# cropinghigh/sdrpp-dvbs-demodulator

Hardware: NVIDIA B200
Metric: decoded_info_gbit_s (higher is better)
Workload: dtype int8

## Files before the change

sdrpp-dvbs-demodulator_b200/csrc/api.cu:

```cuda
#include "../../include/dvbs2fec.h"

#include <algorithm>
#include <atomic>
#include <chrono>
#include <climits>
#include <condition_variable>
#include <cstdarg>
#include <cstdio>
#include <cstring>
#include <deque>
#include <map>
#include <memory>
#include <mutex>
#include <string>
#include <thread>
#include <vector>

#include <cuda_runtime.h>
#include <emmintrin.h>

#include "bch_decoder.cuh"
#include "demapper.cuh"
#include "host_tables.h"
#include "ldpc_decoder.cuh"
// ... 10 lines not shown
    va_start(ap, fmt);
    vsnprintf(g_err, sizeof(g_err), fmt, ap);
    va_end(ap);
    return code;
}
}
namespace s2 {
int api_fail(int code, const char* msg) {
    snprintf(g_err, sizeof(g_err), "%s", msg);
    return code;
}
}
namespace {
#define CU(call)                                                                              \
    do {                                                                                      \
        cudaError_t e_ = (call);                                                              \
        if (e_ != cudaSuccess)                                                                \
            return fail(DVBS2FEC_ECUDA, "%s: %s (%s:%d)", #call, cudaGetErrorString(e_), __FILE__, __LINE__); \
    } while (0)

constexpr int kStages = 4;
constexpr int kPiece = 256;
constexpr int kSlots = 2;

template <typename T>
struct DevBuf {
    T* p = nullptr;
    size_t cap = 0;
    cudaError_t reserve(size_t n) {
        if (n <= cap) return cudaSuccess;
        if (p) cudaFree(p);
        p = nullptr;
        cap = 0;
        cudaError_t e = cudaMalloc(&p, n * sizeof(T));
        if (e == cudaSuccess) cap = n;
        return e;
    }
    void release() {
        if (p) cudaFree(p);
        p = nullptr;
        cap = 0;
    }
};
template <typename T>
struct PinBuf {
    T* p = nullptr;
// ... 12 lines not shown
        p = nullptr;
        cap = 0;
    }
};

struct Slot {
    cudaStream_t stream = nullptr;
    cudaEvent_t done = nullptr;
    cudaStream_t copy = nullptr;
    cudaEvent_t armed = nullptr;
    DevBuf<unsigned int> arrived;
    DevBuf<uint8_t> ts;
    DevBuf<int> ts_len;
    PinBuf<unsigned int> arrived_vals;
    DevBuf<int8_t> llr;
    DevBuf<float> sym;
    DevBuf<uint8_t> idx;
    DevBuf<uint8_t> hard;
    DevBuf<int16_t> iters;
    DevBuf<int16_t> corr;
    DevBuf<uint8_t> bb;
    DevBuf<dvbs2fec_result> res;
    DevBuf<uint8_t> workspace;
    DevBuf<unsigned int> counter;
    PinBuf<uint8_t> h_in;
    PinBuf<uint8_t> h_bb;
    PinBuf<dvbs2fec_result> h_res;
    uint8_t* user_bb = nullptr;
    dvbs2fec_result* user_res = nullptr;
    int pending = 0;
    bool staged_out = true;
    uint64_t tag_base = 0;
};

struct CodeDev {
    DevBuf<uint8_t> row_level;
};
struct BchTabDev {
    DevBuf<uint16_t> crc, basis;
};

struct DevCtx {
    int device = 0;
    int sms = 0;
    Slot slot[2 * kSlots + 1];
    std::mutex dev_mu;
    bool dev_used = false;
    std::map<int, CodeDev> codes;
    std::map<int, BchTabDev> bch;
    DevBuf<uint16_t> gf_log[2], gf_exp[2];
    DevBuf<uint8_t> prbs;
    DevBuf<uint8_t> pl_rn;
    std::map<int, DevBuf<uint32_t>> luts;
    LdpcDev ldpc{};
    BchDev bchd{};
    DemapDev demap{};
    int grid = 0;
    ~DevCtx() { ldpc_release(ldpc); }
};

}

struct dvbs2fec_ts_parser {
    int device = 0;
    int kb = 0, max_dfl = 0;
    cudaStream_t stream = nullptr;
    DevBuf<TsState> state;
    DevBuf<TsPlan> plan;
    DevBuf<uint32_t> meta;
    DevBuf<uint8_t> bb, out;
    PinBuf<int> h_produced;
    int gse_pool = 0;
    DevBuf<GseState> gstate;
    DevBuf<uint8_t> gbuf, g_sync;
    DevBuf<int> g_doff, g_before, g_nxt, g_aux, g_aux2;
// ... 130 lines not shown
    D.lut = nullptr;
    D.rn = h->pl_codenum >= 0 ? d.pl_rn.p : nullptr;
    if (mc.constellation != APSK32) {
        int key = (mc.constellation == APSK16) ? mc.modcod : (int)mc.constellation;
        DevBuf<uint32_t>& lut = d.luts[key];
        if (!lut.p) {
            std::vector<uint32_t> tab = demap_lut(ch);
            CU(lut.reserve(tab.size()));
            CU(cudaMemcpy(lut.p, tab.data(), tab.size() * 4, cudaMemcpyHostToDevice));
            CU(cudaStreamSynchronize(nullptr));
        }
        D.lut = lut.p;
    }
    return 0;
}

size_t input_frame_bytes(const dvbs2fec_handle* h, int kind) {
    return kind == 1 ? (size_t)h->plsyms * 8 : kind == 2 ? (size_t)(h->code->N / h->mc.bits) * 2 : (size_t)h->code->N;
}

int reserve_slot(dvbs2fec_handle* h, DevCtx& d, Slot& s, int nframes, int kind, bool host_staging) {
    const LdpcCode& c = *h->code;
    CU(cudaSetDevice(d.device));
    CU(s.llr.reserve((size_t)nframes * c.N));
    if (kind == 1) CU(s.sym.reserve((size_t)nframes * h->plsyms * 2));
    if (kind == 2) CU(s.idx.reserve((size_t)nframes * input_frame_bytes(h, 2)));
    CU(s.hard.reserve((size_t)nframes * h->hard_stride));
    CU(s.iters.reserve(nframes));
    CU(s.corr.reserve(nframes));
    CU(s.bb.reserve((size_t)nframes * (c.kbch / 8)));
    CU(s.res.reserve(nframes));
    CU(s.workspace.reserve((size_t)d.grid * ldpc_workspace_bytes(d.ldpc)));
    CU(s.counter.reserve(1));
    if (host_staging) {
        size_t in_bytes = (size_t)nframes * input_frame_bytes(h, kind);
        CU(s.h_in.reserve(in_bytes));
        CU(s.h_bb.reserve((size_t)nframes * (c.kbch / 8)));
        CU(s.h_res.reserve(nframes));
    }
    return 0;
}

int enqueue_chain(dvbs2fec_handle* h, DevCtx& d, Slot& s, const float* d_sym, const int8_t* d_llr, int n,
                  uint8_t* d_bb, dvbs2fec_result* d_res, cudaStream_t st, int* launches, uint64_t tag_base = 0,
                  const unsigned int* arrived = nullptr, const uint8_t* d_idx = nullptr) {
    const int8_t* llr = d_llr;
    dvbs2fec_handle::Span cur{0, nullptr, nullptr};
    auto mark = [&](int kind, bool begin) {
        if (!h->profiling) return;
        if (begin) {
            cur = dvbs2fec_handle::Span{kind, nullptr, nullptr};
            cudaEventCreate(&cur.a);
            cudaEventCreate(&cur.b);
            cudaEventRecord(cur.a, st);
        } else {
            cudaEventRecord(cur.b, st);
            std::lock_guard<std::mutex> lk(h->span_mu);
            h->spans.push_back(cur);
        }
    };
    if (d_sym || d_idx) {
        mark(0, true);
        int e = d_sym ? demap_launch(d.demap, d_sym, n, s.llr.p, st) : demap_idx_launch(d.demap, d_idx, n, s.llr.p, st);
        mark(0, false);
        if (e) return fail(DVBS2FEC_ECUDA, "demap launch: %s", cudaGetErrorString((cudaError_t)e));
        llr = s.llr.p;
        ++*launches;
    }
    CU(cudaMemsetAsync(s.counter.p, 0, sizeof(unsigned int), st));
    LdpcArgs la{};
    la.code = d.ldpc;
    la.llr_in = llr;
    la.nframes = n;
    la.max_trials = h->max_trials;
    la.hard_out = s.hard.p;
    la.hard_stride = h->hard_stride;
    la.iters_out = s.iters.p;
    la.llr_out = nullptr;
    la.workspace = s.workspace.p;
    la.work_counter = s.counter.p;
    la.arrived = arrived;
    int grid = std::min(d.grid, (n + 1) / 2);
    mark(1, true);
    int e = ldpc_launch(la, grid, st);
    mark(1, false);
    if (e) return fail(DVBS2FEC_ECUDA, "ldpc launch: %s", cudaGetErrorString((cudaError_t)e));
    ++*launches;
    BchArgs ba{};
    ba.code = d.bchd;
    ba.hard = s.hard.p;
    ba.hard_stride = h->hard_stride;
    ba.nframes = n;
    ba.ldpc_iters = s.iters.p;
    ba.tags = nullptr;
    ba.tag_base = tag_base;
    ba.bb_out = d_bb;
    ba.results = d_res;
    ba.corr_out = nullptr;
    ba.descramble = 1;
    mark(2, true);
    e = bch_launch(ba, st);
    mark(2, false);
    if (e) return fail(DVBS2FEC_ECUDA, "bch launch: %s", cudaGetErrorString((cudaError_t)e));
    ++*launches;
    return 0;
}

int arm_streamed_input(Slot& s, int nframes) {
    CU(s.arrived.reserve(1));
    CU(s.arrived_vals.reserve((size_t)(nframes + kPiece - 1) / kPiece + 1));
    CU(cudaMemsetAsync(s.arrived.p, 0, sizeof(unsigned int), s.copy));
    CU(cudaEventRecord(s.armed, s.copy));
    CU(cudaStreamWaitEvent(s.stream, s.armed, 0));
    return 0;
}
int feed_streamed_input(Slot& s, const uint8_t* src, int nframes, size_t frame_bytes, bool src_pinned) {
    for (int f0 = 0, k = 0; f0 < nframes; f0 += kPiece, ++k) {
        const int n = std::min(kPiece, nframes - f0);
        const uint8_t* from = src + (size_t)f0 * frame_bytes;
        if (!src_pinned) {
            memcpy(s.h_in.p + (size_t)f0 * frame_bytes, from, (size_t)n * frame_bytes);
            from = s.h_in.p + (size_t)f0 * frame_bytes;
        }
        CU(cudaMemcpyAsync(s.llr.p + (size_t)f0 * frame_bytes, from, (size_t)n * frame_bytes, cudaMemcpyHostToDevice, s.copy));
        s.arrived_vals.p[k] = (unsigned int)(f0 + n);
// ... 317 lines not shown
    if (h->worker.joinable()) h->worker.join();
    for (auto& dp : h->devs) {
        DevCtx& d = *dp;
        cudaSetDevice(d.device);
        cudaDeviceSynchronize();
        for (int k = 0; k < 2 * kSlots + 1; ++k) {
            Slot& s = d.slot[k];
            s.llr.release(); s.sym.release(); s.idx.release(); s.hard.release(); s.iters.release(); s.corr.release();
            s.bb.release(); s.res.release(); s.workspace.release(); s.counter.release();
            s.h_in.release(); s.h_bb.release(); s.h_res.release();
            s.arrived.release(); s.arrived_vals.release();
            s.ts.release(); s.ts_len.release();
            if (s.done) cudaEventDestroy(s.done);
            if (s.armed) cudaEventDestroy(s.armed);
            if (s.copy && !(k >= 1 && k < kSlots)) cudaStreamDestroy(s.copy);
            if (s.stream) cudaStreamDestroy(s.stream);
        }
        for (auto& kv : d.codes) kv.second.row_level.release();
        for (auto& kv : d.bch) { kv.second.crc.release(); kv.second.basis.release(); }
        for (auto& kv : d.luts) kv.second.release();
        for (int i = 0; i < 2; ++i) { d.gf_log[i].release(); d.gf_exp[i].release(); }
        d.prbs.release();
        d.pl_rn.release();
    }
    if (h->ts) dvbs2fec_ts_destroy(h->ts);
    if (h->ts_done) cudaEventDestroy(h->ts_done);
    for (auto& sp : h->spans) {
        cudaEventDestroy(sp.a);
        cudaEventDestroy(sp.b);
    }
    for (auto& S : h->stages) {
        S.in.release();
        S.bb.release();
        S.res.release();
        S.ts.release();
        S.ts_len.release();
    }
    delete h;
}

int dvbs2fec_set_modcod(dvbs2fec_handle* h, int modcod, int shortframes, int pilots, int max_trials) {
    if (!h) return fail(DVBS2FEC_EINVAL, "handle is NULL");
    ModcodCfg mc;
    if (!modcod_config(modcod, shortframes != 0, pilots != 0, &mc))
        return fail(DVBS2FEC_EINVAL, "MODCOD %d is outside 1..28", modcod);
    if (mc.code < 0)
// ... 25 lines not shown
    if (codenum > 262141) return fail(DVBS2FEC_EINVAL, "Gold code number %d outside 0..262141", codenum);
    drain_queue(h);
    h->pl_codenum = codenum < 0 ? -1 : codenum;
    for (auto& dp : h->devs) {
        DevCtx& d = *dp;
        CU(cudaSetDevice(d.device));
        if (codenum >= 0) {
            std::vector<uint8_t> rn = pl_scrambling_rn(codenum, 32400 + 36 * 22 + 8);
            CU(d.pl_rn.reserve(rn.size()));
            CU(cudaMemcpy(d.pl_rn.p, rn.data(), rn.size(), cudaMemcpyHostToDevice));
            CU(cudaStreamSynchronize(nullptr));
        }
        d.demap.rn = codenum >= 0 ? d.pl_rn.p : nullptr;
    }
    return 0;
}

int dvbs2fec_kbch(const dvbs2fec_handle* h) { return (h && h->configured) ? h->code->kbch : DVBS2FEC_EINVAL; }
int dvbs2fec_kldpc(const dvbs2fec_handle* h) { return (h && h->configured) ? h->code->K : DVBS2FEC_EINVAL; }
int dvbs2fec_nldpc(const dvbs2fec_handle* h) { return (h && h->configured) ? h->code->N : DVBS2FEC_EINVAL; }
int dvbs2fec_plframe_symbols(const dvbs2fec_handle* h) { return (h && h->configured) ? h->plsyms : DVBS2FEC_EINVAL; }
int dvbs2fec_last_launch_count(const dvbs2fec_handle* h) { return h ? h->last_launches : 0; }

int dvbs2fec_set_profiling(dvbs2fec_handle* h, int on) {
    if (!h) return fail(DVBS2FEC_EINVAL, "handle is NULL");
    h->profiling = on != 0;
    return 0;
}
int dvbs2fec_kernel_times(dvbs2fec_handle* h, float* demap_ms, float* ldpc_ms, float* bch_ms, int* launches) {
    if (!h) return fail(DVBS2FEC_EINVAL, "handle is NULL");
    float acc[3] = {0, 0, 0};
    int n = 0;
    std::vector<dvbs2fec_handle::Span> spans;
    {
        std::lock_guard<std::mutex> lk(h->span_mu);
        spans.swap(h->spans);
    }
    for (auto& sp : spans) {
        float ms = 0;
        CU(cudaEventSynchronize(sp.b));
        CU(cudaEventElapsedTime(&ms, sp.a, sp.b));
        acc[sp.kind] += ms;
        cudaEventDestroy(sp.a);
        cudaEventDestroy(sp.b);
        ++n;
    }
    if (demap_ms) *demap_ms = acc[0];
    if (ldpc_ms) *ldpc_ms = acc[1];
    if (bch_ms) *bch_ms = acc[2];
    if (launches) *launches = n;
    return 0;
}

int dvbs2fec_bb_to_soft(dvbs2fec_handle* h, const float* plframes, int n, int8_t* llr_out) {
    if (!h || !h->configured || !plframes || !llr_out || n < 0) return fail(DVBS2FEC_EINVAL, "bad arguments");
    if (n == 0) return 0;
    DevCtx& d = *h->devs[0];
    Slot& s = d.slot[0];
    int rc = reserve_slot(h, d, s, n, 1, false);
    if (rc) return rc;
    CU(cudaMemcpyAsync(s.sym.p, plframes, (size_t)n * h->plsyms * 8, cudaMemcpyHostToDevice, s.stream));
    int e = demap_launch(d.demap, s.sym.p, n, s.llr.p, s.stream);
    if (e) return fail(DVBS2FEC_ECUDA, "demap launch: %s", cudaGetErrorString((cudaError_t)e));
    CU(cudaMemcpyAsync(llr_out, s.llr.p, (size_t)n * h->code->N, cudaMemcpyDeviceToHost, s.stream));
    CU(cudaStreamSynchronize(s.stream));
    return 0;
}

int dvbs2fec_ldpc_decode(dvbs2fec_handle* h, int8_t* frames, int n, int max_trials, int16_t* iters) {
    if (!h || !h->configured || !frames || n < 0) return fail(DVBS2FEC_EINVAL, "bad arguments");
    if (n == 0) return 0;
    DevCtx& d = *h->devs[0];
    Slot& s = d.slot[0];
    int rc = reserve_slot(h, d, s, n, 0, false);
    if (rc) return rc;
    const size_t bytes = (size_t)n * h->code->N;
    CU(cudaMemcpyAsync(s.llr.p, frames, bytes, cudaMemcpyHostToDevice, s.stream));
    CU(cudaMemsetAsync(s.counter.p, 0, sizeof(unsigned int), s.stream));
    LdpcArgs la{};
    la.code = d.ldpc;
    la.llr_in = s.llr.p;
    la.nframes = n;
    la.max_trials = max_trials > 0 ? max_trials : h->max_trials;
    la.hard_out = s.hard.p;
    la.hard_stride = h->hard_stride;
    la.iters_out = s.iters.p;
    la.llr_out = s.llr.p;
    la.workspace = s.workspace.p;
    la.work_counter = s.counter.p;
    la.arrived = nullptr;
    int e = ldpc_launch(la, std::min(d.grid, (n + 1) / 2), s.stream);
    if (e) return fail(DVBS2FEC_ECUDA, "ldpc launch: %s", cudaGetErrorString((cudaError_t)e));
    CU(cudaMemcpyAsync(frames, s.llr.p, bytes, cudaMemcpyDeviceToHost, s.stream));
    if (iters) CU(cudaMemcpyAsync(iters, s.iters.p, (size_t)n * 2, cudaMemcpyDeviceToHost, s.stream));
    CU(cudaStreamSynchronize(s.stream));
    return 0;
}

int dvbs2fec_bch_decode(dvbs2fec_handle* h, uint8_t* frames, int n, int16_t* corrections) {
    if (!h || !h->configured || !frames || n < 0) return fail(DVBS2FEC_EINVAL, "bad arguments");
    if (n == 0) return 0;
    DevCtx& d = *h->devs[0];
    Slot& s = d.slot[0];
    int rc = reserve_slot(h, d, s, n, 0, false);
    if (rc) return rc;
    const size_t nb = h->code->K / 8;
    CU(cudaMemsetAsync(s.hard.p, 0, (size_t)n * h->hard_stride, s.stream));
    CU(cudaMemcpy2DAsync(s.hard.p, h->hard_stride, frames, nb, nb, n, cudaMemcpyHostToDevice, s.stream));
    BchArgs ba{};
    ba.code = d.bchd;
    ba.hard = s.hard.p;
    ba.hard_stride = h->hard_stride;
    ba.nframes = n;
    ba.corr_out = s.corr.p;
    int e = bch_launch(ba, s.stream);
// ... 616 lines not shown
```

sdrpp-dvbs-demodulator_b200/csrc/bch_decoder.cu:

```cuda
#include "bch_decoder.cuh"

namespace s2 {
namespace {

constexpr int kWarps = 4;
constexpr int kMaxT = 12;

struct ResultRec {
    unsigned long long tag;
    short ldpc_iters;
    short bch_corr;
    unsigned int flags;
};

__device__ __forceinline__ uint32_t gf_mul(const GfDev& f, uint32_t a, uint32_t b) {
    if (!a || !b) return 0;
    int s = (int)f.log[a] + (int)f.log[b];
    if (s >= f.N) s -= f.N;
    return f.exp[s];
}
__device__ __forceinline__ uint32_t gf_div(const GfDev& f, uint32_t a, uint32_t b) {
    if (!a) return 0;
    int s = (int)f.log[a] - (int)f.log[b];
    if (s < 0) s += f.N;
    return f.exp[s];
}
__device__ __forceinline__ uint32_t gf_mul_exp(const GfDev& f, uint32_t a, int e) {
    if (!a) return 0;
    int s = (int)f.log[a] + e;
    if (s >= f.N) s -= f.N;
    return f.exp[s];
}

__device__ __forceinline__ uint32_t warp_xor(uint32_t v) {
#pragma unroll
    for (int o = 16; o; o >>= 1) v ^= __shfl_xor_sync(0xFFFFFFFFu, v, o);
    return v;
}

__global__ void __launch_bounds__(kWarps * 32) bch_kernel(const __grid_constant__ BchArgs a) {
    extern __shared__ __align__(16) uint8_t smem[];
    const BchDev& c = a.code;
    const GfDev& f = c.gf;
    const int t = c.t, NR = 2 * c.t, m = f.m;
    uint16_t* s_crc = reinterpret_cast<uint16_t*>(smem);
    uint16_t* s_basis = s_crc + kMaxT * 256;
    uint8_t* s_frames = reinterpret_cast<uint8_t*>(s_basis + kMaxT * 16);
    const int wid = threadIdx.x >> 5, lane = threadIdx.x & 31;
    uint8_t* fr = s_frames + (size_t)wid * a.hard_stride;
    __shared__ uint16_t s_synd[kWarps][24];
    __shared__ uint16_t s_lambda[kWarps][26];
    __shared__ uint16_t s_ev[kWarps][26];
    __shared__ int s_loc[kWarps][26];
    __shared__ int s_nloc[kWarps];

    for (int x = threadIdx.x; x < t * 256; x += blockDim.x) s_crc[x] = c.crc[x];
    for (int x = threadIdx.x; x < t * 16; x += blockDim.x) s_basis[x] = c.basis[x];
    __syncthreads();

    const int nbytes = c.nbch >> 3, kbytes = c.kbch >> 3;
    for (int frame = blockIdx.x * kWarps + wid; frame < a.nframes; frame += gridDim.x * kWarps) {
        uint8_t* gfr = a.hard + (size_t)frame * a.hard_stride;
        for (int x = lane; x < a.hard_stride / 16; x += 32)
            reinterpret_cast<uint4*>(fr)[x] = reinterpret_cast<const uint4*>(gfr)[x];
        __syncwarp();

        const int chunk = (nbytes + 31) >> 5;
        const int beg = min(lane * chunk, nbytes), end = min(beg + chunk, nbytes);
        uint32_t r[kMaxT];
#pragma unroll
        for (int k = 0; k < kMaxT; ++k) r[k] = 0;
        const uint32_t rmask = (1u << m) - 1u;
        for (int x = beg; x < end; ++x) {
            uint32_t byte = fr[x];
#pragma unroll
            for (int k = 0; k < kMaxT; ++k)
                if (k < t) {
                    uint32_t idx = r[k] >> (m - 8);
// ... 172 lines not shown
            int it = a.ldpc_iters ? a.ldpc_iters[frame] : 0;
            if (a.corr_out) a.corr_out[frame] = (int16_t)corr;
            if (a.results) {
                ResultRec rr;
                rr.tag = a.tags ? a.tags[frame] : a.tag_base + (unsigned long long)frame;
                rr.ldpc_iters = (short)it;
                rr.bch_corr = (short)corr;
                rr.flags = (it < 0 ? 1u : 0u) | (corr < 0 ? 2u : 0u);
                if (a.descramble) {
                    uint32_t crc = 0;
                    for (int n = 0; n < 80; ++n) {
                        uint32_t byte = fr[n >> 3] ^ c.prbs[n >> 3];
                        uint32_t b = ((byte >> (7 - (n & 7))) & 1u) ^ (crc & 1u);
                        crc >>= 1;
                        if (b) crc ^= 0xABu;
                    }
                    if (crc) rr.flags |= 4u;
                }
                reinterpret_cast<ResultRec*>(a.results)[frame] = rr;
            }
        }
        __syncwarp();
    }
}

__global__ void descramble_kernel(uint8_t* frames, int stride, int nframes, int kbytes, const uint8_t* prbs) {
    int x = blockIdx.x * blockDim.x + threadIdx.x;
    int f = blockIdx.y;
    if (x < kbytes && f < nframes) frames[(size_t)f * stride + x] ^= prbs[x];
}

}

int bch_launch(const BchArgs& a, cudaStream_t stream) {
    if (a.nframes <= 0) return 0;
    if (a.code.t > kMaxT || (a.hard_stride & 15)) return (int)cudaErrorInvalidValue;
    size_t smem = (size_t)kMaxT * 256 * 2 + kMaxT * 16 * 2 + (size_t)kWarps * a.hard_stride;
    int grid = (a.nframes + kWarps - 1) / kWarps;
    if (grid > 148 * 16) grid = 148 * 16;
    bch_kernel<<<grid, kWarps * 32, smem, stream>>>(a);
    return (int)cudaGetLastError();
}

int descramble_launch(uint8_t* frames, int stride, int nframes, int kbch, const uint8_t* prbs, cudaStream_t stream) {
    if (nframes <= 0) return 0;
    int kbytes = kbch / 8;
    dim3 grid((kbytes + 255) / 256, nframes);
    descramble_kernel<<<grid, 256, 0, stream>>>(frames, stride, nframes, kbytes, prbs);
    return (int)cudaGetLastError();
}

}
```

sdrpp-dvbs-demodulator_b200/csrc/bch_decoder.cuh:

```cuda
#pragma once
#include <cstdint>
#include <cuda_runtime.h>

namespace s2 {

struct GfDev {
    int m, N;
    const uint16_t* log;
    const uint16_t* exp;
};

struct BchDev {
    GfDev gf;
    int t;
    int nbch, kbch;
    int prefix;
    const uint16_t* crc;
    const uint16_t* basis;
    const uint8_t* prbs;
};

struct BchArgs {
    BchDev code;
    uint8_t* hard;
    int hard_stride;
    int nframes;
    const int16_t* ldpc_iters;
    const uint64_t* tags;
    unsigned long long tag_base;
    uint8_t* bb_out;
    void* results;
    int16_t* corr_out;
    int descramble;
};

int bch_launch(const BchArgs& args, cudaStream_t stream);

int descramble_launch(uint8_t* frames, int stride, int nframes, int kbch, const uint8_t* prbs, cudaStream_t stream);

}
```

sdrpp-dvbs-demodulator_b200/csrc/ldpc_decoder.cu:

```cuda
#include "ldpc_decoder.cuh"
#include "ldpc_variants.h"

#include <algorithm>
#include <cstdio>
#include <cstdlib>
#include <cstring>
#include <vector>

namespace s2 {

struct LdpcPlan {
    bool v2 = false;
    int threads = kLdpcThreads;
    KernelFn fn1[2] = {nullptr, nullptr};
    KernelFn2 fn2[2] = {nullptr, nullptr};
    LdpcParams p1;
    LdpcParams2 p2;
    size_t smem = 0;
};

namespace {

int env_int(const char* name, int dflt) {
    const char* e = getenv(name);
// ... 217 lines not shown
void ldpc_release(LdpcDev& c) {
    delete c.plan;
    c.plan = nullptr;
}

int ldpc_max_ctas_per_sm(const LdpcDev& c) {
    if (!c.plan) return 0;
    int n = 0;
    if (c.plan->v2)
        cudaOccupancyMaxActiveBlocksPerMultiprocessor(&n, c.plan->fn2[0], c.plan->threads, c.plan->smem);
    else
        cudaOccupancyMaxActiveBlocksPerMultiprocessor(&n, c.plan->fn1[0], kLdpcThreads, c.plan->smem);
    return n;
}

int ldpc_launch(const LdpcArgs& a, int grid, cudaStream_t stream) {
    const LdpcPlan* pl = a.code.plan;
    if (!pl) return (int)cudaErrorInvalidValue;
    const int st = a.arrived ? 1 : 0;
    if (pl->v2) {
        LdpcParams2 p = pl->p2;
        p.nframes = a.nframes; p.max_trials = a.max_trials; p.hard_stride = a.hard_stride;
        p.llr_in = a.llr_in; p.hard_out = a.hard_out; p.iters_out = a.iters_out; p.llr_out = a.llr_out;
        p.workspace = a.workspace; p.work_counter = a.work_counter; p.arrived = a.arrived;
        pl->fn2[st]<<<grid, pl->threads, pl->smem, stream>>>(p);
    } else {
        LdpcParams p = pl->p1;
        p.nframes = a.nframes; p.max_trials = a.max_trials; p.hard_stride = a.hard_stride;
        p.llr_in = a.llr_in; p.hard_out = a.hard_out; p.iters_out = a.iters_out; p.llr_out = a.llr_out;
        p.workspace = a.workspace; p.work_counter = a.work_counter; p.arrived = a.arrived;
        pl->fn1[st]<<<grid, kLdpcThreads, pl->smem, stream>>>(p);
    }
    return (int)cudaGetLastError();
}

}
```

sdrpp-dvbs-demodulator_b200/csrc/ldpc_decoder.cuh:

```cuda
#pragma once
#include <cstdint>
#include <cuda_runtime.h>

namespace s2 {

constexpr int kLdpcThreads = 384;
constexpr int kBitWords = 13;
constexpr int16_t kLdpcItersNoInput = -2;

struct LdpcPlan;

struct LdpcDev {
    int N, K, R, q;
    int ngroups;
    int max_cnt;
    int sg;
    bool chains;
    bool occ3;
    bool v2;
    bool lanes2;
    const LdpcPlan* plan;
    const uint32_t* links;
    const int* layer_off;
    const uint8_t* layer_nlev;
    const uint8_t* row_level;
};
int ldpc_slot_groups(int max_cnt);
bool ldpc_chains_pay_off(int code_index);
bool ldpc_ctas_wanted3(int code_index);
bool ldpc_use_v2(int code_index);
bool ldpc_use_lanes2(int code_index);
int ldpc_slot_groups_for(int max_cnt, bool lanes2);
int ldpc_prepare(LdpcDev& code);
void ldpc_release(LdpcDev& code);

struct LdpcArgs {
    LdpcDev code;
    const int8_t* llr_in;
    int nframes;
    int max_trials;
    uint8_t* hard_out;
    int hard_stride;
    int16_t* iters_out;
    int8_t* llr_out;
    uint8_t* workspace;
    unsigned int* work_counter;
    const unsigned int* arrived;
};

inline size_t ldpc_workspace_bytes(const LdpcDev& c) {
    size_t b = (size_t)c.q * c.sg * 360 * 16 + (((size_t)c.R * 2 + 15) & ~(size_t)15);
    if (c.v2) b += (size_t)2 * (c.ngroups + c.q) * kBitWords * 4 + 32 + (size_t)768 * 16;
    return (b + 255) & ~(size_t)255;
}
inline size_t ldpc_smem_bytes(const LdpcDev& c) {
    if (c.v2 && c.lanes2) return (size_t)c.K * 2 + 768 + (size_t)c.q * (4 + 2 * ((2 * ((c.max_cnt + 1) / 2) + 3) & ~3)) * 4 + 64;
    if (c.v2) return (size_t)c.K * 2 + 768 + (size_t)c.q * ((1 + 2 * c.max_cnt + 3) & ~3) * 4 + 64;
    const size_t base = (size_t)c.K * 2 + (size_t)2 * (c.ngroups + c.q) * kBitWords * 4;
    return c.chains ? ((base + 15) & ~(size_t)15) + 360 * 16 + 64 : base + 64;
}

int ldpc_launch(const LdpcArgs& args, int grid, cudaStream_t stream);
int ldpc_max_ctas_per_sm(const LdpcDev& code);

}
```

sdrpp-dvbs-demodulator_b200/csrc/ldpc_kernels.cuh:

```cuda
#pragma once
#include "ldpc_decoder.cuh"
#include "ldpc_variants.h"

namespace s2 {
namespace {


__device__ __forceinline__ uint32_t prmt(uint32_t a, uint32_t b, uint32_t sel) {
    uint32_t d;
    asm("prmt.b32 %0, %1, %2, %3;" : "=r"(d) : "r"(a), "r"(b), "r"(sel));
    return d;
}
__device__ __forceinline__ uint32_t unpack01(uint32_t w) { return prmt(w, 0, 0x9180); }
__device__ __forceinline__ uint32_t unpack23(uint32_t w) { return prmt(w, 0, 0xB3A2); }
__device__ __forceinline__ uint32_t pack1(uint32_t x) { return prmt(x, 0, 0x4420); }
__device__ __forceinline__ uint32_t pack2(uint32_t x0, uint32_t x1) { return prmt(x0, x1, 0x6420); }

constexpr uint32_t kM128 = 0xFF80FF80u, kP127 = 0x007F007Fu, kP32 = 0x00200020u, kP31 = 0x001F001Fu;
constexpr uint32_t kM1 = 0xFFFFFFFFu, kBig = 0x7FFF7FFFu;

__device__ __forceinline__ uint32_t sat8x2(uint32_t x) { return __vmins2(__vmaxs2(x, kM128), kP127); }

__device__ __forceinline__ uint32_t zero_bytes(uint32_t w) {
    return ~(((w & 0x7F7Fu) + 0x7F7Fu) | w) & 0x8080u;
// ... 254 lines not shown
    }
}

template <int CNT, bool UNIFORM, bool STREAMED, bool CHAINS, int OCC = (CNT <= 9 ? 2 : 1)>
__global__ void __launch_bounds__(kLdpcThreads, OCC) ldpc_pair_kernel(const __grid_constant__ LdpcParams p) {
    constexpr int SLOTS = CNT + 2;
    constexpr int MW = (SLOTS + 1) / 2;
    constexpr int SG = (SLOTS + 7) / 8;
    extern __shared__ __align__(16) uint8_t smem_raw[];
    uint16_t* vdata = reinterpret_cast<uint16_t*>(smem_raw);
    uint32_t* HD = reinterpret_cast<uint32_t*>(smem_raw + (size_t)p.K * 2);
    uint32_t* HP = HD + 2 * p.ngroups * kBitWords;
    __shared__ unsigned int s_pair;
    __shared__ int s_bad[2];

    const int tid = threadIdx.x, lane = tid & 31, wid = tid >> 5;
    const int j = tid;
    const bool active = j < 360;
    const int q = p.q, K = p.K, N = p.N, R = p.R;
    uint4* wmsg = reinterpret_cast<uint4*>(p.workspace + (size_t)blockIdx.x * p.ws_stride);
    uint16_t* wpty = reinterpret_cast<uint16_t*>(p.workspace + (size_t)blockIdx.x * p.ws_stride +
                                                 (size_t)q * SG * 360 * 16);
    const int npairs = (p.nframes + 1) >> 1;
    uint4* chain_scratch = reinterpret_cast<uint4*>(smem_raw + ((((size_t)K * 2 + (size_t)2 * (p.ngroups + q) * kBitWords * 4) + 15) & ~(size_t)15));

    for (int x = tid; x < 2 * (p.ngroups + q) * kBitWords; x += kLdpcThreads) HD[x] = 0;

    for (;;) {
        __syncthreads();
        if (tid == 0) {
            const unsigned np = atomicAdd(p.work_counter, 1u);
            s_pair = np;
            if (STREAMED && np < (unsigned)npairs) {
                wait_arrived(p.arrived, min(2u * np + 2u, (unsigned)p.nframes));
                __threadfence();
            }
        }
        __syncthreads();
        const unsigned pair = s_pair;
        if (pair >= (unsigned)npairs) break;
        const int fa = 2 * pair, fb = 2 * pair + 1;
        const bool hasB = fb < p.nframes;
        const int8_t* inA = p.llr_in + (size_t)fa * N;
        const int8_t* inB = p.llr_in + (size_t)(hasB ? fb : fa) * N;

        for (int x = tid; x < K / 8; x += kLdpcThreads) {
            uint2 a = STREAMED ? __ldcg(reinterpret_cast<const uint2*>(inA) + x) : __ldg(reinterpret_cast<const uint2*>(inA) + x);
            uint2 b = STREAMED ? __ldcg(reinterpret_cast<const uint2*>(inB) + x) : __ldg(reinterpret_cast<const uint2*>(inB) + x);
            uint4 o;
            o.x = prmt(a.x, b.x, 0x5140) ^ 0x80808080u;
            o.y = prmt(a.x, b.x, 0x7362) ^ 0x80808080u;
            o.z = prmt(a.y, b.y, 0x5140) ^ 0x80808080u;
            o.w = prmt(a.y, b.y, 0x7362) ^ 0x80808080u;
            reinterpret_cast<uint4*>(vdata)[x] = o;
// ... 205 lines not shown
        const int kbytes = K / 8;
        for (int x = tid; x < 2 * kbytes; x += kLdpcThreads) {
            int f = x >= kbytes, b = x - f * kbytes;
            if (f && !hasB) break;
            int g = b / 45, k = b - g * 45;
            uint32_t word = HD[(f * p.ngroups + g) * kBitWords + (k >> 2)];
            uint32_t byte = (word >> (8 * (k & 3))) & 0xFFu;
            p.hard_out[(size_t)(f ? fb : fa) * p.hard_stride + b] = (uint8_t)(__brev(byte) >> 24);
        }
        if (p.llr_out) {
            for (int x = tid; x < K; x += kLdpcThreads) {
                uint32_t v = vdata[x] ^ 0x8080u;
                p.llr_out[(size_t)fa * N + x] = (int8_t)(v & 0xFF);
                if (hasB) p.llr_out[(size_t)fb * N + x] = (int8_t)(v >> 8);
            }
            for (int x = tid; x < R; x += kLdpcThreads) {
                int jj = x / q, ii = x - jj * q;
                uint32_t v = __ldcg(&wpty[360 * ii + jj]) ^ 0x8080u;
                p.llr_out[(size_t)fa * N + K + x] = (int8_t)(v & 0xFF);
                if (hasB) p.llr_out[(size_t)fb * N + K + x] = (int8_t)(v >> 8);
            }
        }
    }
}

}
}

#define K2(c, u, st, ch) {ldpc_pair_kernel<c, u, st, ch>, ldpc_pair_kernel<c, u, st, ch, (c <= 9 ? 3 : 2)>}
#define K8(c, u) {{K2(c, u, false, false), K2(c, u, false, true)}, {K2(c, u, true, false), K2(c, u, true, true)}}
#define N8 {{{nullptr, nullptr}, {nullptr, nullptr}}, {{nullptr, nullptr}, {nullptr, nullptr}}}
#define VU(c) {c, K8(c, true), N8}
#define VB(c) {c, K8(c, true), K8(c, false)}
#define VR(c) {c, N8, K8(c, false)}
```

sdrpp-dvbs-demodulator_b200/csrc/ldpc_v2.cuh:

```cuda
#pragma once
#include "ldpc_decoder.cuh"
#include "ldpc_variants.h"

#include <type_traits>

namespace s2 {
namespace v2 {

constexpr int kThreads = 360;

__device__ __forceinline__ uint32_t prmt(uint32_t a, uint32_t b, uint32_t sel) {
    uint32_t d;
    asm("prmt.b32 %0, %1, %2, %3;" : "=r"(d) : "r"(a), "r"(b), "r"(sel));
    return d;
}
__device__ __forceinline__ uint32_t minu2(uint32_t a, uint32_t b) {
    uint32_t d;
    asm("min.u16x2 %0, %1, %2;" : "=r"(d) : "r"(a), "r"(b));
    return d;
}
__device__ __forceinline__ uint32_t min3u2(uint32_t a, uint32_t b, uint32_t c) {
    uint32_t d;
    asm("{.reg .b32 t; min.u16x2 t, %1, %2; min.u16x2 %0, t, %3;}" : "=r"(d) : "r"(a), "r"(b), "r"(c));
    return d;
// ... 284 lines not shown
    uint4* wmsg = reinterpret_cast<uint4*>(p.workspace + (size_t)blockIdx.x * p.ws_stride);
    uint16_t* wpty = reinterpret_cast<uint16_t*>(p.workspace + (size_t)blockIdx.x * p.ws_stride + (size_t)q * SG * 360 * 16);
    uint32_t* HD = reinterpret_cast<uint32_t*>(reinterpret_cast<uint8_t*>(wpty) + (((size_t)R * 2 + 15) & ~(size_t)15));
    uint32_t* HP = HD + 2 * p.ngroups * kBitWords;
    {
        volatile uint4* opq = reinterpret_cast<volatile uint4*>(HP + 2 * q * kBitWords + 4) + tid;
        opq->x = j2; opq->y = xaddr; opq->z = dbase; opq->w = m1;
        j2 = opq->x; xaddr = opq->y; dbase = opq->z; m1 = opq->w;
    }
    for (int x = tid; x < q * DW; x += kThreads) {
        const int i = x / DW, w = x - i * DW;
        const int loff = p.layer_off[i], cnt = (int)p.layer_off[i + 1] - loff;
        uint32_t v = 0;
        if (w == 0) {
            v = (uint32_t)p.layer_nlev[i] | (uint32_t)p.layer_sync[i] << 8 | (uint32_t)cnt << 16;
        } else if (w <= 2 * CNT) {
            const int c = (w - 1) >> 1;
            const int k = loff + (c < cnt ? c : 0);
            v = ((w - 1) & 1) ? (uint32_t)p.link_add[k] : vbase + 720u * p.link_group[k];
        }
        desc[x] = v;
    }
    const int npairs = (p.nframes + 1) >> 1;

    for (int x = tid; x < 2 * (p.ngroups + q) * kBitWords; x += kThreads) __stcg(&HD[x], 0u);

    for (;;) {
        __syncthreads();
        if (tid == 0) {
            unsigned np = atomicAdd(p.work_counter, 1u);
            if (STREAMED && np < (unsigned)npairs) {
                if (!wait_arrived(p.arrived, min(2u * np + 2u, (unsigned)p.nframes), p.wait_budget)) np |= 0x80000000u;
                __threadfence();
            }
            s_pair = np;
        }
        __syncthreads();
        const unsigned pair_word = s_pair;
        const unsigned pair = pair_word & 0x7FFFFFFFu;
        if (pair >= (unsigned)npairs) break;
        const int fa = 2 * pair, fb = 2 * pair + 1;
        const bool hasB = fb < p.nframes;
        if (STREAMED && (pair_word & 0x80000000u)) {
            if (tid == 0) {
                p.iters_out[fa] = kLdpcItersNoInput;
                if (hasB) p.iters_out[fb] = kLdpcItersNoInput;
            }
            continue;
        }
        const int8_t* inA = p.llr_in + (size_t)fa * N;
        const int8_t* inB = p.llr_in + (size_t)(hasB ? fb : fa) * N;
        const int8_t* colA = inA + K + (size_t)q * j;
        const int8_t* colB = inB + K + (size_t)q * j;
// ... 155 lines not shown
                        sts_u16(xaddr, pack_pair(psec));
                    else
                        __stcg(pp - 360, (uint16_t)pack_pair(psec));
                    pprev = psec;
                    psec = pown;
                    rp += SG * 360;
                    pp += 360;
                    ca += 1;
                    cb += 1;
                }
                psec = pprev;
                {
                    const uint16_t pk = (uint16_t)pack_pair(pown);
                    sts_u16(xaddr + 2, pk);
                    __stcg(pp - 360, pk);
                }
            };
            if (n == 0) pass(std::true_type{});
            else pass(std::false_type{});
            __syncthreads();
            scr = screen();
        }
    }
}

}
}

#define S2_V2_K4(c, r) {{v2::ldpc_v2_kernel<c, r, false, (c <= 9 ? 2 : 1)>, v2::ldpc_v2_kernel<c, r, false, (c <= 9 ? 3 : 2)>}, \
                        {v2::ldpc_v2_kernel<c, r, true, (c <= 9 ? 2 : 1)>, v2::ldpc_v2_kernel<c, r, true, (c <= 9 ? 3 : 2)>}}
#define S2_V2_N4 {{nullptr, nullptr}, {nullptr, nullptr}}
#define V2U(c) {c, S2_V2_K4(c, false), S2_V2_N4}
#define V2B(c) {c, S2_V2_K4(c, false), S2_V2_K4(c, true)}
#define V2R(c) {c, S2_V2_N4, S2_V2_K4(c, true)}
```

sdrpp-dvbs-demodulator_b200/csrc/ldpc_v2l.cuh:

```cuda
#pragma once
#include "ldpc_v2.cuh"

namespace s2 {
namespace v2 {

constexpr int kLdpcThreads2 = 720;

template <int NL, bool FIRST, bool RAGGED>
__device__ __forceinline__ void row_update2(const uint32_t (&off)[NL], int cntl, uint32_t (&mw)[(NL + 2) / 2], uint32_t& preg,
                                            uint32_t keep, uint32_t m1, unsigned lanes) {
    constexpr int DH = NL + 1;
    uint32_t tu[DH], a[DH];
    uint32_t sx = ((2 * DH - 1) & 1) ? kC128 : 0u;
#pragma unroll
    for (int s = 0; s < DH; ++s) {
        uint32_t u;
        if (s == 0)
            u = preg;
        else
            u = (!RAGGED || s - 1 < cntl) ? unpack_lo(lds_u16(off[s - 1])) : kC255;
        uint32_t t = u;
        if (!FIRST) {
            const uint32_t beta = (s & 1) ? unpack_hi(mw[s >> 1]) : unpack_lo(mw[s >> 1]);
            t = addmin_relu(u + beta, kM32, kC255);
// ... 76 lines not shown
    uint32_t* HP = HD + 2 * p.ngroups * kBitWords;
    {
        volatile uint4* opq = reinterpret_cast<volatile uint4*>(HP + 2 * q * kBitWords + 4) + tid;
        opq->x = j2; opq->y = xaddr; opq->z = dbase; opq->w = m1;
        j2 = opq->x; xaddr = opq->y; dbase = opq->z; m1 = opq->w;
    }
    for (int x = tid; x < q * DW; x += T) {
        const int i = x / DW, w = x - i * DW;
        const int loff = p.layer_off[i], cnt = (int)p.layer_off[i + 1] - loff;
        uint32_t v = 0;
        if (w == 0) {
            v = (uint32_t)p.layer_nlev[i] | (uint32_t)p.layer_sync[i] << 8 | (uint32_t)cnt << 16;
        } else if (w >= 4) {
            const int hh = (w - 4) / HW, e = (w - 4) - hh * HW;
            const int s = e >> 1, d = 2 * s + hh;
            if (s < NL) {
                const int k = loff + (d < cnt ? d : 0);
                v = (e & 1) ? (uint32_t)p.link_add[k] : vbase + 720u * p.link_group[k];
            }
        }
        desc[x] = v;
    }
    const int npairs = (p.nframes + 1) >> 1;
    for (int x = tid; x < 2 * (p.ngroups + q) * kBitWords; x += T) __stcg(&HD[x], 0u);

    for (;;) {
        __syncthreads();
        if (tid == 0) {
            unsigned np = atomicAdd(p.work_counter, 1u);
            if (STREAMED && np < (unsigned)npairs) {
                if (!wait_arrived(p.arrived, min(2u * np + 2u, (unsigned)p.nframes), p.wait_budget)) np |= 0x80000000u;
                __threadfence();
            }
            s_pair = np;
        }
        __syncthreads();
        const unsigned pair_word = s_pair;
        const unsigned pair = pair_word & 0x7FFFFFFFu;
        if (pair >= (unsigned)npairs) break;
        const int fa = 2 * pair, fb = 2 * pair + 1;
        const bool hasB = fb < p.nframes;
        if (STREAMED && (pair_word & 0x80000000u)) {
            if (tid == 0) {
                p.iters_out[fa] = kLdpcItersNoInput;
                if (hasB) p.iters_out[fb] = kLdpcItersNoInput;
            }
            continue;
        }
        const int8_t* inA = p.llr_in + (size_t)fa * N;
        const int8_t* inB = p.llr_in + (size_t)(hasB ? fb : fa) * N;
        const int8_t* colA = inA + K + (size_t)q * j;
        const int8_t* colB = inB + K + (size_t)q * j;
// ... 161 lines not shown
                            sts_u16(xaddr, pack_pair(preg));
                        else
                            __stcg(pp - 360, (uint16_t)pack_pair(preg));
                    }
                    const uint32_t other = __shfl_xor_sync(wl, preg, 1);
                    if (h == 1 && i + 1 < q) preg = other;
                    rp += 2 * SG * 360;
                    pp += 360;
                    ca += 1;
                    cb += 1;
                }
                if (h == 0) {
                    const uint16_t pk = (uint16_t)pack_pair(preg);
                    sts_u16(xaddr + 2, pk);
                    __stcg(pp - 360, pk);
                }
            };
            if (n == 0) pass(std::true_type{});
            else pass(std::false_type{});
            __syncthreads();
            scr = screen();
        }
    }
}

}
}

#define S2_V2L_K2(c, r) {v2::ldpc_v2l_kernel<c, r, false>, v2::ldpc_v2l_kernel<c, r, true>}
#define S2_V2L_N2 {nullptr, nullptr}
#define V2LU(c) {c, S2_V2L_K2(c, false), S2_V2L_N2}
#define V2LR(c) {c, S2_V2L_N2, S2_V2L_K2(c, true)}
```

sdrpp-dvbs-demodulator_b200/csrc/ldpc_variants.h:

```cpp
#pragma once
#include <cstdint>

namespace s2 {

constexpr int kMaxLinks = 656;
constexpr int kMaxLayers = 136;
struct LdpcParams {
    int N, K, R, q, ngroups, sg;
    int nframes, max_trials, hard_stride, pad_;
    const int8_t* llr_in;
    uint8_t* hard_out;
    int16_t* iters_out;
    int8_t* llr_out;
    uint8_t* workspace;
    unsigned long long ws_stride;
    unsigned int* work_counter;
    const unsigned int* arrived;
    const uint8_t* row_level;
    uint16_t layer_off[kMaxLayers + 1];
    uint8_t layer_nlev[kMaxLayers];
    uint8_t layer_sync[kMaxLayers];
    uint16_t layer_chain[kMaxLayers];
    uint32_t links[kMaxLinks];
};
static_assert(sizeof(LdpcParams) <= 4096, "kernel parameter block must stay within the 4 KB constant window");

using KernelFn = void (*)(const LdpcParams);
struct Variant {
    int cnt;
    KernelFn uniform[2][2][2];
    KernelFn ragged[2][2][2];
};
extern const Variant kLdpcVariantsA[], kLdpcVariantsB[], kLdpcVariantsC[], kLdpcVariantsD[];
extern const int kLdpcVariantsA_n, kLdpcVariantsB_n, kLdpcVariantsC_n, kLdpcVariantsD_n;

struct LdpcParams2 {
    int N, K, R, q, ngroups, sg;
    int nframes, max_trials, hard_stride, pad_;
    long long wait_budget;
    const int8_t* llr_in;
    uint8_t* hard_out;
    int16_t* iters_out;
    int8_t* llr_out;
    uint8_t* workspace;
    unsigned long long ws_stride;
    unsigned int* work_counter;
    const unsigned int* arrived;
    const uint8_t* row_level;
    uint16_t layer_off[kMaxLayers + 1];
    uint8_t layer_nlev[kMaxLayers];
    uint8_t layer_sync[kMaxLayers];
    uint8_t link_group[kMaxLinks];
    uint16_t link_add[kMaxLinks];
};
static_assert(sizeof(LdpcParams2) <= 4096, "kernel parameter block must stay within the 4 KB constant window");

using KernelFn2 = void (*)(const LdpcParams2);
struct Variant2 {
    int cnt;
    KernelFn2 uniform[2][2];
    KernelFn2 ragged[2][2];
};
extern const Variant2 kLdpc2VariantsA[], kLdpc2VariantsB[], kLdpc2VariantsC[], kLdpc2VariantsD[];
extern const int kLdpc2VariantsA_n, kLdpc2VariantsB_n, kLdpc2VariantsC_n, kLdpc2VariantsD_n;

struct VariantL {
    int cnt;
    KernelFn2 uniform[2];
    KernelFn2 ragged[2];
// ... 6 lines not shown
```

Before: 22.21.

## Replace per-launch counter memset with monotonic work counter; template BCH on t

The per-launch cudaMemsetAsync that reset the LDPC work counter is removed. Instead a 64-bit monotonic counter is kept per slot, and each launch passes a host-tracked pair_base to subtract, which saves one stream operation per chain. The BCH kernel is now templated on the correction capability t, so NR and t loops are compile-time constants, and it gets a minimum-blocks launch bound. Profiling switches from cudaEvent spans to in-kernel globaltimer stamps, which adds a null-pointer check in each kernel.

```diff
diff --git a/sdrpp-dvbs-demodulator_b200/csrc/api.cu b/sdrpp-dvbs-demodulator_b200/csrc/api.cu
--- a/sdrpp-dvbs-demodulator_b200/csrc/api.cu
+++ b/sdrpp-dvbs-demodulator_b200/csrc/api.cu
@@ -56,6 +56,7 @@
 constexpr int kStages = 4;
 constexpr int kPiece = 256;
 constexpr int kSlots = 2;
+constexpr int kStampCalls = 4096;
 
 template <typename T>
 struct DevBuf {
@@ -114,7 +115,8 @@
     DevBuf<uint8_t> bb;
     DevBuf<dvbs2fec_result> res;
     DevBuf<uint8_t> workspace;
-    DevBuf<unsigned int> counter;
+    DevBuf<unsigned long long> counter;
+    unsigned long long taken = 0;
     PinBuf<uint8_t> h_in;
     PinBuf<uint8_t> h_bb;
     PinBuf<dvbs2fec_result> h_res;
@@ -143,6 +145,8 @@
     DevBuf<uint16_t> gf_log[2], gf_exp[2];
     DevBuf<uint8_t> prbs;
     DevBuf<uint8_t> pl_rn;
+    DevBuf<unsigned long long> stamps;
+    int stamps_used = 0;
     std::map<int, DevBuf<uint32_t>> luts;
     LdpcDev ldpc{};
     BchDev bchd{};
@@ -319,6 +323,12 @@
 int reserve_slot(dvbs2fec_handle* h, DevCtx& d, Slot& s, int nframes, int kind, bool host_staging) {
     const LdpcCode& c = *h->code;
     CU(cudaSetDevice(d.device));
+    if (!s.counter.p) {
+        CU(s.counter.reserve(1));
+        CU(cudaMemset(s.counter.p, 0, sizeof(unsigned long long)));
+        CU(cudaStreamSynchronize(nullptr));
+        s.taken = 0;
+    }
     CU(s.llr.reserve((size_t)nframes * c.N));
     if (kind == 1) CU(s.sym.reserve((size_t)nframes * h->plsyms * 2));
     if (kind == 2) CU(s.idx.reserve((size_t)nframes * input_frame_bytes(h, 2)));
@@ -328,7 +338,6 @@
     CU(s.bb.reserve((size_t)nframes * (c.kbch / 8)));
     CU(s.res.reserve(nframes));
     CU(s.workspace.reserve((size_t)d.grid * ldpc_workspace_bytes(d.ldpc)));
-    CU(s.counter.reserve(1));
     if (host_staging) {
         size_t in_bytes = (size_t)nframes * input_frame_bytes(h, kind);
         CU(s.h_in.reserve(in_bytes));
@@ -336,6 +345,13 @@
         CU(s.h_res.reserve(nframes));
     }
     return 0;
+}
+
+unsigned long long* take_stamps(dvbs2fec_handle* h, DevCtx& d) {
+    if (!h->profiling) return nullptr;
+    std::lock_guard<std::mutex> lk(h->span_mu);
+    if (!d.stamps.p || d.stamps_used >= kStampCalls) return nullptr;
+    return d.stamps.p + (size_t)kStampWords * d.stamps_used++;
 }
 
 int enqueue_chain(dvbs2fec_handle* h, DevCtx& d, Slot& s, const float* d_sym, const int8_t* d_llr, int n,
@@ -364,7 +380,7 @@
         llr = s.llr.p;
         ++*launches;
     }
-    CU(cudaMemsetAsync(s.counter.p, 0, sizeof(unsigned int), st));
+    unsigned long long* stamps = take_stamps(h, d);
     LdpcArgs la{};
     la.code = d.ldpc;
     la.llr_in = llr;
@@ -376,12 +392,13 @@
     la.llr_out = nullptr;
     la.workspace = s.workspace.p;
     la.work_counter = s.counter.p;
+    la.pair_base = s.taken;
+    la.stamps = stamps;
     la.arrived = arrived;
     int grid = std::min(d.grid, (n + 1) / 2);
-    mark(1, true);
     int e = ldpc_launch(la, grid, st);
-    mark(1, false);
     if (e) return fail(DVBS2FEC_ECUDA, "ldpc launch: %s", cudaGetErrorString((cudaError_t)e));
+    s.taken += (unsigned long long)((n + 1) / 2 + grid);
     ++*launches;
     BchArgs ba{};
     ba.code = d.bchd;
@@ -395,9 +412,8 @@
     ba.results = d_res;
     ba.corr_out = nullptr;
     ba.descramble = 1;
-    mark(2, true);
+    ba.stamps = stamps;
     e = bch_launch(ba, st);
-    mark(2, false);
     if (e) return fail(DVBS2FEC_ECUDA, "bch launch: %s", cudaGetErrorString((cudaError_t)e));
     ++*launches;
     return 0;
@@ -761,6 +777,7 @@
         for (int i = 0; i < 2; ++i) { d.gf_log[i].release(); d.gf_exp[i].release(); }
         d.prbs.release();
         d.pl_rn.release();
+        d.stamps.release();
     }
     if (h->ts) dvbs2fec_ts_destroy(h->ts);
     if (h->ts_done) cudaEventDestroy(h->ts_done);
@@ -832,8 +849,31 @@
 int dvbs2fec_plframe_symbols(const dvbs2fec_handle* h) { return (h && h->configured) ? h->plsyms : DVBS2FEC_EINVAL; }
 int dvbs2fec_last_launch_count(const dvbs2fec_handle* h) { return h ? h->last_launches : 0; }
 
+namespace {
+int reset_stamps(dvbs2fec_handle* h) {
+    static std::vector<unsigned long long> blank = [] {
+        std::vector<unsigned long long> v((size_t)kStampCalls * kStampWords, 0ull);
+        for (size_t i = 0; i < v.size(); i += kStampWords) v[i] = v[i + 2] = ~0ull;
+        return v;
+    }();
+    for (auto& dp : h->devs) {
+        DevCtx& d = *dp;
+        CU(cudaSetDevice(d.device));
+        CU(d.stamps.reserve(blank.size()));
+        CU(cudaMemcpy(d.stamps.p, blank.data(), blank.size() * sizeof(unsigned long long), cudaMemcpyHostToDevice));
+        CU(cudaStreamSynchronize(nullptr));
+        d.stamps_used = 0;
+    }
+    return 0;
+}
+}
+
 int dvbs2fec_set_profiling(dvbs2fec_handle* h, int on) {
     if (!h) return fail(DVBS2FEC_EINVAL, "handle is NULL");
+    if (on && !h->profiling) {
+        std::lock_guard<std::mutex> lk(h->span_mu);
+        if (int rc = reset_stamps(h)) return rc;
+    }
     h->profiling = on != 0;
     return 0;
 }
@@ -855,6 +895,24 @@
         cudaEventDestroy(sp.b);
         ++n;
     }
+    std::lock_guard<std::mutex> lk(h->span_mu);
+    for (auto& dp : h->devs) {
+        DevCtx& d = *dp;
+        if (!d.stamps_used) continue;
+        std::vector<unsigned long long> st((size_t)d.stamps_used * kStampWords);
+        CU(cudaSetDevice(d.device));
+        CU(cudaDeviceSynchronize());
+        CU(cudaMemcpy(st.data(), d.stamps.p, st.size() * sizeof(unsigned long long), cudaMemcpyDeviceToHost));
+        for (size_t i = 0; i < st.size(); i += kStampWords)
+            for (int k = 0; k < 2; ++k)
+                if (st[i + 2 * k] != ~0ull && st[i + 2 * k + 1] >= st[i + 2 * k]) {
+                    acc[1 + k] += (float)((st[i + 2 * k + 1] - st[i + 2 * k]) * 1e-6);
+                    ++n;
+                }
+    }
+    for (auto& dp : h->devs) dp->stamps_used = 0;
+    if (h->profiling)
+        if (int rc = reset_stamps(h)) return rc;
     if (demap_ms) *demap_ms = acc[0];
     if (ldpc_ms) *ldpc_ms = acc[1];
     if (bch_ms) *bch_ms = acc[2];
@@ -886,7 +944,6 @@
     if (rc) return rc;
     const size_t bytes = (size_t)n * h->code->N;
     CU(cudaMemcpyAsync(s.llr.p, frames, bytes, cudaMemcpyHostToDevice, s.stream));
-    CU(cudaMemsetAsync(s.counter.p, 0, sizeof(unsigned int), s.stream));
     LdpcArgs la{};
     la.code = d.ldpc;
     la.llr_in = s.llr.p;
@@ -898,9 +955,12 @@
     la.llr_out = s.llr.p;
     la.workspace = s.workspace.p;
     la.work_counter = s.counter.p;
+    la.pair_base = s.taken;
     la.arrived = nullptr;
-    int e = ldpc_launch(la, std::min(d.grid, (n + 1) / 2), s.stream);
+    const int grid = std::min(d.grid, (n + 1) / 2);
+    int e = ldpc_launch(la, grid, s.stream);
     if (e) return fail(DVBS2FEC_ECUDA, "ldpc launch: %s", cudaGetErrorString((cudaError_t)e));
+    s.taken += (unsigned long long)((n + 1) / 2 + grid);
     CU(cudaMemcpyAsync(frames, s.llr.p, bytes, cudaMemcpyDeviceToHost, s.stream));
     if (iters) CU(cudaMemcpyAsync(iters, s.iters.p, (size_t)n * 2, cudaMemcpyDeviceToHost, s.stream));
     CU(cudaStreamSynchronize(s.stream));
diff --git a/sdrpp-dvbs-demodulator_b200/csrc/bch_decoder.cu b/sdrpp-dvbs-demodulator_b200/csrc/bch_decoder.cu
--- a/sdrpp-dvbs-demodulator_b200/csrc/bch_decoder.cu
+++ b/sdrpp-dvbs-demodulator_b200/csrc/bch_decoder.cu
@@ -38,11 +38,14 @@
     return v;
 }
 
-__global__ void __launch_bounds__(kWarps * 32) bch_kernel(const __grid_constant__ BchArgs a) {
+template <int T>
+__global__ void __launch_bounds__(kWarps * 32, 6) bch_kernel(const __grid_constant__ BchArgs a) {
     extern __shared__ __align__(16) uint8_t smem[];
     const BchDev& c = a.code;
     const GfDev& f = c.gf;
-    const int t = c.t, NR = 2 * c.t, m = f.m;
+    static_assert(T <= kMaxT, "at most kMaxT corrections");
+    constexpr int t = T, NR = 2 * T;
+    const int m = f.m;
     uint16_t* s_crc = reinterpret_cast<uint16_t*>(smem);
     uint16_t* s_basis = s_crc + kMaxT * 256;
     uint8_t* s_frames = reinterpret_cast<uint8_t*>(s_basis + kMaxT * 16);
@@ -54,6 +57,7 @@
     __shared__ int s_loc[kWarps][26];
     __shared__ int s_nloc[kWarps];
 
+    if (a.stamps && threadIdx.x == 0) atomicMin(&a.stamps[2], globaltimer());
     for (int x = threadIdx.x; x < t * 256; x += blockDim.x) s_crc[x] = c.crc[x];
     for (int x = threadIdx.x; x < t * 16; x += blockDim.x) s_basis[x] = c.basis[x];
     __syncthreads();
@@ -272,6 +276,10 @@
         }
         __syncwarp();
     }
+    if (a.stamps) {
+        __syncthreads();
+        if (threadIdx.x == 0) atomicMax(&a.stamps[3], globaltimer());
+    }
 }
 
 __global__ void descramble_kernel(uint8_t* frames, int stride, int nframes, int kbytes, const uint8_t* prbs) {
@@ -288,7 +296,12 @@
     size_t smem = (size_t)kMaxT * 256 * 2 + kMaxT * 16 * 2 + (size_t)kWarps * a.hard_stride;
     int grid = (a.nframes + kWarps - 1) / kWarps;
     if (grid > 148 * 16) grid = 148 * 16;
-    bch_kernel<<<grid, kWarps * 32, smem, stream>>>(a);
+    switch (a.code.t) {
+    case 8: bch_kernel<8><<<grid, kWarps * 32, smem, stream>>>(a); break;
+    case 10: bch_kernel<10><<<grid, kWarps * 32, smem, stream>>>(a); break;
+    case 12: bch_kernel<12><<<grid, kWarps * 32, smem, stream>>>(a); break;
+    default: return (int)cudaErrorInvalidValue;
+    }
     return (int)cudaGetLastError();
 }
 
diff --git a/sdrpp-dvbs-demodulator_b200/csrc/bch_decoder.cuh b/sdrpp-dvbs-demodulator_b200/csrc/bch_decoder.cuh
--- a/sdrpp-dvbs-demodulator_b200/csrc/bch_decoder.cuh
+++ b/sdrpp-dvbs-demodulator_b200/csrc/bch_decoder.cuh
@@ -1,6 +1,8 @@
 #pragma once
 #include <cstdint>
 #include <cuda_runtime.h>
+
+#include "stamps.cuh"
 
 namespace s2 {
 
@@ -32,6 +34,7 @@
     void* results;
     int16_t* corr_out;
     int descramble;
+    unsigned long long* stamps;
 };
 
 int bch_launch(const BchArgs& args, cudaStream_t stream);
diff --git a/sdrpp-dvbs-demodulator_b200/csrc/ldpc_decoder.cu b/sdrpp-dvbs-demodulator_b200/csrc/ldpc_decoder.cu
--- a/sdrpp-dvbs-demodulator_b200/csrc/ldpc_decoder.cu
+++ b/sdrpp-dvbs-demodulator_b200/csrc/ldpc_decoder.cu
@@ -263,13 +263,15 @@
         LdpcParams2 p = pl->p2;
         p.nframes = a.nframes; p.max_trials = a.max_trials; p.hard_stride = a.hard_stride;
         p.llr_in = a.llr_in; p.hard_out = a.hard_out; p.iters_out = a.iters_out; p.llr_out = a.llr_out;
-        p.workspace = a.workspace; p.work_counter = a.work_counter; p.arrived = a.arrived;
+        p.workspace = a.workspace; p.work_counter = a.work_counter; p.pair_base = a.pair_base; p.stamps = a.stamps;
+        p.arrived = a.arrived;
         pl->fn2[st]<<<grid, pl->threads, pl->smem, stream>>>(p);
     } else {
         LdpcParams p = pl->p1;
         p.nframes = a.nframes; p.max_trials = a.max_trials; p.hard_stride = a.hard_stride;
         p.llr_in = a.llr_in; p.hard_out = a.hard_out; p.iters_out = a.iters_out; p.llr_out = a.llr_out;
-        p.workspace = a.workspace; p.work_counter = a.work_counter; p.arrived = a.arrived;
+        p.workspace = a.workspace; p.work_counter = a.work_counter; p.pair_base = a.pair_base; p.stamps = a.stamps;
+        p.arrived = a.arrived;
         pl->fn1[st]<<<grid, kLdpcThreads, pl->smem, stream>>>(p);
     }
     return (int)cudaGetLastError();
diff --git a/sdrpp-dvbs-demodulator_b200/csrc/ldpc_decoder.cuh b/sdrpp-dvbs-demodulator_b200/csrc/ldpc_decoder.cuh
--- a/sdrpp-dvbs-demodulator_b200/csrc/ldpc_decoder.cuh
+++ b/sdrpp-dvbs-demodulator_b200/csrc/ldpc_decoder.cuh
@@ -1,6 +1,8 @@
 #pragma once
 #include <cstdint>
 #include <cuda_runtime.h>
+
+#include "stamps.cuh"
 
 namespace s2 {
 
@@ -44,7 +46,9 @@
     int16_t* iters_out;
     int8_t* llr_out;
     uint8_t* workspace;
-    unsigned int* work_counter;
+    unsigned long long* work_counter;
+    unsigned long long pair_base;
+    unsigned long long* stamps;
     const unsigned int* arrived;
 };
 
diff --git a/sdrpp-dvbs-demodulator_b200/csrc/ldpc_kernels.cuh b/sdrpp-dvbs-demodulator_b200/csrc/ldpc_kernels.cuh
--- a/sdrpp-dvbs-demodulator_b200/csrc/ldpc_kernels.cuh
+++ b/sdrpp-dvbs-demodulator_b200/csrc/ldpc_kernels.cuh
@@ -300,6 +300,7 @@
     uint16_t* wpty = reinterpret_cast<uint16_t*>(p.workspace + (size_t)blockIdx.x * p.ws_stride +
                                                  (size_t)q * SG * 360 * 16);
     const int npairs = (p.nframes + 1) >> 1;
+    if (p.stamps && tid == 0) atomicMin(&p.stamps[0], globaltimer());
     uint4* chain_scratch = reinterpret_cast<uint4*>(smem_raw + ((((size_t)K * 2 + (size_t)2 * (p.ngroups + q) * kBitWords * 4) + 15) & ~(size_t)15));
 
     for (int x = tid; x < 2 * (p.ngroups + q) * kBitWords; x += kLdpcThreads) HD[x] = 0;
@@ -307,7 +308,8 @@
     for (;;) {
         __syncthreads();
         if (tid == 0) {
-            const unsigned np = atomicAdd(p.work_counter, 1u);
+            const unsigned long long c = atomicAdd(p.work_counter, 1ull) - p.pair_base;
+            const unsigned np = c < (unsigned long long)npairs ? (unsigned)c : (unsigned)npairs;
             s_pair = np;
             if (STREAMED && np < (unsigned)npairs) {
                 wait_arrived(p.arrived, min(2u * np + 2u, (unsigned)p.nframes));
@@ -559,6 +561,7 @@
             }
         }
     }
+    if (p.stamps && tid == 0) atomicMax(&p.stamps[1], globaltimer());
 }
 
 }
diff --git a/sdrpp-dvbs-demodulator_b200/csrc/ldpc_v2.cuh b/sdrpp-dvbs-demodulator_b200/csrc/ldpc_v2.cuh
--- a/sdrpp-dvbs-demodulator_b200/csrc/ldpc_v2.cuh
+++ b/sdrpp-dvbs-demodulator_b200/csrc/ldpc_v2.cuh
@@ -330,13 +330,15 @@
         desc[x] = v;
     }
     const int npairs = (p.nframes + 1) >> 1;
+    if (p.stamps && tid == 0) atomicMin(&p.stamps[0], globaltimer());
 
     for (int x = tid; x < 2 * (p.ngroups + q) * kBitWords; x += kThreads) __stcg(&HD[x], 0u);
 
     for (;;) {
         __syncthreads();
         if (tid == 0) {
-            unsigned np = atomicAdd(p.work_counter, 1u);
+            const unsigned long long c = atomicAdd(p.work_counter, 1ull) - p.pair_base;
+            unsigned np = c < (unsigned long long)npairs ? (unsigned)c : (unsigned)npairs;
             if (STREAMED && np < (unsigned)npairs) {
                 if (!wait_arrived(p.arrived, min(2u * np + 2u, (unsigned)p.nframes), p.wait_budget)) np |= 0x80000000u;
                 __threadfence();
@@ -538,6 +540,7 @@
             scr = screen();
         }
     }
+    if (p.stamps && tid == 0) atomicMax(&p.stamps[1], globaltimer());
 }
 
 }
diff --git a/sdrpp-dvbs-demodulator_b200/csrc/ldpc_v2l.cuh b/sdrpp-dvbs-demodulator_b200/csrc/ldpc_v2l.cuh
--- a/sdrpp-dvbs-demodulator_b200/csrc/ldpc_v2l.cuh
+++ b/sdrpp-dvbs-demodulator_b200/csrc/ldpc_v2l.cuh
@@ -122,12 +122,14 @@
         desc[x] = v;
     }
     const int npairs = (p.nframes + 1) >> 1;
+    if (p.stamps && tid == 0) atomicMin(&p.stamps[0], globaltimer());
     for (int x = tid; x < 2 * (p.ngroups + q) * kBitWords; x += T) __stcg(&HD[x], 0u);
 
     for (;;) {
         __syncthreads();
         if (tid == 0) {
-            unsigned np = atomicAdd(p.work_counter, 1u);
+            const unsigned long long c = atomicAdd(p.work_counter, 1ull) - p.pair_base;
+            unsigned np = c < (unsigned long long)npairs ? (unsigned)c : (unsigned)npairs;
             if (STREAMED && np < (unsigned)npairs) {
                 if (!wait_arrived(p.arrived, min(2u * np + 2u, (unsigned)p.nframes), p.wait_budget)) np |= 0x80000000u;
                 __threadfence();
@@ -335,6 +337,7 @@
             scr = screen();
         }
     }
+    if (p.stamps && tid == 0) atomicMax(&p.stamps[1], globaltimer());
 }
 
 }
diff --git a/sdrpp-dvbs-demodulator_b200/csrc/ldpc_variants.h b/sdrpp-dvbs-demodulator_b200/csrc/ldpc_variants.h
--- a/sdrpp-dvbs-demodulator_b200/csrc/ldpc_variants.h
+++ b/sdrpp-dvbs-demodulator_b200/csrc/ldpc_variants.h
@@ -1,5 +1,7 @@
 #pragma once
 #include <cstdint>
+
+#include "stamps.cuh"
 
 namespace s2 {
 
@@ -14,7 +16,9 @@
     int8_t* llr_out;
     uint8_t* workspace;
     unsigned long long ws_stride;
-    unsigned int* work_counter;
+    unsigned long long* work_counter;
+    unsigned long long pair_base;
+    unsigned long long* stamps;
     const unsigned int* arrived;
     const uint8_t* row_level;
     uint16_t layer_off[kMaxLayers + 1];
@@ -44,7 +48,9 @@
     int8_t* llr_out;
     uint8_t* workspace;
     unsigned long long ws_stride;
-    unsigned int* work_counter;
+    unsigned long long* work_counter;
+    unsigned long long pair_base;
+    unsigned long long* stamps;
     const unsigned int* arrived;
     const uint8_t* row_level;
     uint16_t layer_off[kMaxLayers + 1];
diff --git a/sdrpp-dvbs-demodulator_b200/csrc/stamps.cuh b/sdrpp-dvbs-demodulator_b200/csrc/stamps.cuh
--- /dev/null
+++ b/sdrpp-dvbs-demodulator_b200/csrc/stamps.cuh
@@ -0,0 +1,15 @@
+#pragma once
+
+namespace s2 {
+
+constexpr int kStampWords = 4;
+
+#ifdef __CUDACC__
+__device__ __forceinline__ unsigned long long globaltimer() {
+    unsigned long long t;
+    asm volatile("mov.u64 %0, %%globaltimer;" : "=l"(t));
+    return t;
+}
+#endif
+
+}
```

Measured after the change: 22.72 (median of 6 runs). +2.3%, better.
